# cruiseresearchgroup/ViLCo

Hardware: AMD Instinct MI355X
Metric: clips/sec (fwd+bwd) MQ transformer T=2304 C=2304 (higher is better)
Workload: dtype fp16 MFMA on 2-part splits of power-of-two scaled fp32 operands (22 significant bits, 3 MFMAs per product), fp32 accumulate: fp32-equivalent; weight-gradient products with contraction length >= 2048 use the leading fp16 parts only (11-bit operands, 1 MFMA; <= 3.5e-4 of the 3-MFMA gradients at this c; 1 GPU; MQ ViLCo backbone config P: T=2304 Cin=2304 D=1024 H=16 arch(2,2,5) XLNet layer text L=77x768 22 classes, train mode with the reference's dropout 0.1 / droppath 0.1 / XLNet dropout 0.1 (mq_vilco.yaml, xlnet_config_1024.json); clips_per_gpu=2, global_batch=2, parallelism=dp1

## Files before the change

include/vilco_hip.h:

```cpp
#ifndef VILCO_HIP_H
#define VILCO_HIP_H

#include <stddef.h>
#include <stdint.h>

#ifdef __cplusplus
extern "C" {
#endif

enum vilco_status {
  VILCO_OK = 0,
  VILCO_ERR_BADARG = -1,
  VILCO_ERR_UNSUPPORTED = -2,
  VILCO_ERR_LAUNCH = -3,
  VILCO_ERR_WORKSPACE = -4
};

const char* vilco_status_str(int status);
const char* vilco_version(void);
int vilco_sync_timeouts_read(void);

enum { VILCO_ACT_NONE = 0, VILCO_ACT_RELU = 1, VILCO_ACT_GELU = 2 };
enum { VILCO_TAP_NONE = 0, VILCO_TAP_A = 1, VILCO_TAP_B = 2 };

typedef struct vilco_gemm_desc {
  const float* A;
  const float* B;
  float* C;
  int32_t M, N, K;
  int32_t a_kcontig;
  int32_t b_kcontig;
  int64_t lda, ldb, ldc;
  int32_t batch_outer, batch_inner;
  int64_t sAo, sAi, sBo, sBi, sCo, sCi;
  int32_t tap_operand, tapC, tapT;
  int32_t precision;
  float alpha, beta;
  const float* bias;
  float* preact;
  int32_t act;
  const int32_t* row_len;
  int32_t rowT;
  const float* colscale;
  const float* residual;
  int32_t res_masked;
  void* workspace;
  size_t workspace_bytes;
  const void* a_planes;
  const void* b_planes;
  int32_t band, bandT;
  float drop_p;
  uint32_t drop_seed;
  float* amax_out;
  const float* a_amax; int32_t a_namax;
  const float* b_amax; int32_t b_namax;
  int32_t a_planes_seq, b_planes_seq;
  const float* row_mask;
} vilco_gemm_desc;

size_t vilco_gemm_workspace(const vilco_gemm_desc* d);
int vilco_gemm(const vilco_gemm_desc* d, void* stream);
int vilco_gemm_group(const vilco_gemm_desc* descs, int32_t n, void* stream);

int vilco_gemm_force(int32_t bm, int32_t ks);
int vilco_gemm_set_fixup(int32_t on);
int vilco_gemm_set_gl(int32_t on);
int vilco_gemm_set_tail128(int32_t on);
int vilco_gemm_set_skinny(int32_t on);
int64_t vilco_gemm_config_gen(void);
int32_t vilco_gemm_amax_parts(const vilco_gemm_desc* desc);
int vilco_gemm_profile_begin(void);
int vilco_gemm_profile_end(double* kernel_ms, int64_t* launches);
int64_t vilco_gemm_profile_records(int64_t* desc, double* ms, int64_t cap);

size_t vilco_pack_bytes(int64_t rows, int64_t cols, int32_t precision);
int vilco_pack(const float* src, int64_t rows, int64_t cols, int64_t ld, int32_t precision, void* planes,
               size_t planes_bytes, void* stream);
typedef struct vilco_pack_item {
  const float* src;
  int64_t rows, cols, ld;
  void* planes;
  size_t planes_bytes;
  int32_t nbatch;
  int64_t batch_stride;
  int32_t relshift;
  const float* amax;
  int32_t namax;
  int32_t seq_len;
} vilco_pack_item;
size_t vilco_pack_item_bytes(const vilco_pack_item* item, int32_t precision);
int vilco_pack_many(const vilco_pack_item* items, int32_t n, int32_t precision, void* stream);

int vilco_layernorm_fwd(const float* x, const float* gamma, const float* beta, float* y,
                        float* mean, float* rstd, int64_t rows, int32_t C, float eps,
                        int32_t relu, void* stream);
int vilco_layernorm_fwd_amax(const float* x, const float* gamma, const float* beta, float* y,
                             float* mean, float* rstd, int64_t rows, int32_t C, float eps,
                             int32_t relu, float* amax_parts, int32_t* n_parts, void* stream);
size_t vilco_layernorm_planes_bytes(int64_t rows, int32_t C, int32_t seq_len);
int vilco_layernorm_fwd_planes(const float* x, const float* gamma, const float* beta, float* y,
                               float* mean, float* rstd, int64_t rows, int32_t C, float eps,
                               int32_t relu, float* amax_parts, int32_t* n_parts, void* planes, size_t planes_bytes,
                               int32_t seq_len, const float* row_mask, int64_t mask_rows, void* stream);
size_t vilco_layernorm_bwd_workspace(int64_t rows, int32_t C);
int vilco_layernorm_bwd(const float* dy, const float* x, const float* y, const float* gamma,
                        const float* mean, const float* rstd, float* dx, float* dgamma,
                        float* dbeta, int64_t rows, int32_t C, int32_t relu, void* workspace,
                        size_t workspace_bytes, void* stream);
int vilco_layernorm_bwd_res(const float* dy, const float* x, const float* y, const float* gamma,
                            const float* mean, const float* rstd, const float* dres, float* dx, float* dgamma,
                            float* dbeta, int64_t rows, int32_t C, int32_t relu, void* workspace,
                            size_t workspace_bytes, void* stream);
int vilco_layernorm_bwd_res_amax(const float* dy, const float* x, const float* y, const float* gamma,
                                 const float* mean, const float* rstd, const float* dres, float* dx, float* dgamma,
                                 float* dbeta, int64_t rows, int32_t C, int32_t relu, void* workspace,
                                 size_t workspace_bytes, float* dx_amax_parts, int32_t* n_parts, void* stream);

int vilco_dwconv3_fwd(const float* x, const float* w, const int32_t* in_len, float* y, int32_t B,
                      int32_t Tin, int32_t C, int32_t stride, void* stream);
size_t vilco_dwconv3_bwd_workspace(int32_t B, int32_t Tin, int32_t C, int32_t stride);
int vilco_dwconv3_bwd(const float* dy, const float* x, const float* w, const int32_t* in_len,
// ... 201 lines not shown
```

vilco_amd/_lib.py:

```python
import ctypes as C
import os

_HERE = os.path.dirname(os.path.abspath(__file__))
LIB_PATH = os.environ.get("VILCO_HIP_LIB") or os.path.join(_HERE, "libvilco_hip.so")

ACT_NONE, ACT_RELU, ACT_GELU = 0, 1, 2
TAP_NONE, TAP_A, TAP_B = 0, 1, 2

c_fp = C.c_void_p
i32, i64, f32, sz = C.c_int32, C.c_int64, C.c_float, C.c_size_t


class GemmDesc(C.Structure):
    _fields_ = [
        ("A", c_fp), ("B", c_fp), ("C", c_fp),
        ("M", i32), ("N", i32), ("K", i32),
        ("a_kcontig", i32), ("b_kcontig", i32),
        ("lda", i64), ("ldb", i64), ("ldc", i64),
        ("batch_outer", i32), ("batch_inner", i32),
        ("sAo", i64), ("sAi", i64), ("sBo", i64), ("sBi", i64), ("sCo", i64), ("sCi", i64),
        ("tap_operand", i32), ("tapC", i32), ("tapT", i32),
        ("precision", i32),
        ("alpha", f32), ("beta", f32),
        ("bias", c_fp), ("preact", c_fp), ("act", i32),
        ("row_len", c_fp), ("rowT", i32),
        ("colscale", c_fp), ("residual", c_fp), ("res_masked", i32),
        ("workspace", c_fp), ("workspace_bytes", sz),
        ("a_planes", c_fp), ("b_planes", c_fp),
        ("band", i32), ("bandT", i32),
        ("drop_p", f32), ("drop_seed", C.c_uint32),
        ("amax_out", c_fp),
        ("a_amax", c_fp), ("a_namax", i32), ("b_amax", c_fp), ("b_namax", i32),
        ("a_planes_seq", i32), ("b_planes_seq", i32),
        ("row_mask", c_fp),
    ]


class LossDesc(C.Structure):
    _fields_ = [("logits", c_fp), ("offsets", c_fp), ("level_scale", c_fp), ("points", c_fp), ("row_level", c_fp),
                ("row_pos", c_fp), ("level_len", c_fp), ("gt", c_fp), ("gauss", c_fp), ("loss_norm", c_fp),
                ("B", i32), ("R", i32), ("C", i32), ("L", i32), ("Nmax", i32),
                ("center_radius", f32), ("label_smoothing", f32), ("momentum", f32), ("loss_weight", f32),
                ("al_weight", f32), ("use_al", i32)]


class AttnAmaxIn(C.Structure):
    _fields_ = [("q", c_fp), ("nq", i32), ("k", c_fp), ("nk", i32), ("v", c_fp), ("nv", i32), ("dout", c_fp), ("ndo", i32)]


class PackItem(C.Structure):
    _fields_ = [("src", c_fp), ("rows", i64), ("cols", i64), ("ld", i64), ("planes", c_fp), ("planes_bytes", sz),
                ("nbatch", i32), ("batch_stride", i64), ("relshift", i32), ("amax", c_fp), ("namax", i32), ("seq_len", i32)]


SIGNATURES = {
    "vilco_status_str": (C.c_char_p, [C.c_int]),
    "vilco_version": (C.c_char_p, []),
    "vilco_sync_timeouts_read": (C.c_int, []),
    "vilco_defer_set": (C.c_int, [i32]),
    "vilco_defer_pending": (i64, []),
    "vilco_defer_flush": (C.c_int, [c_fp]),
    "vilco_gemm_workspace": (sz, [C.POINTER(GemmDesc)]),
    "vilco_gemm": (C.c_int, [C.POINTER(GemmDesc), c_fp]),
    "vilco_gemm_group": (C.c_int, [C.POINTER(GemmDesc), i32, c_fp]),
    "vilco_gemm_amax_parts": (i32, [C.POINTER(GemmDesc)]),
    "vilco_gemm_force": (C.c_int, [i32, i32]),
    "vilco_gemm_set_fixup": (C.c_int, [i32]),
    "vilco_gemm_set_gl": (C.c_int, [i32]),
    "vilco_gemm_set_tail128": (C.c_int, [i32]),
    "vilco_gemm_set_skinny": (C.c_int, [i32]),
    "vilco_gemm_config_gen": (i64, []),
    "vilco_gemm_profile_begin": (C.c_int, []),
    "vilco_gemm_profile_end": (C.c_int, [C.POINTER(C.c_double), C.POINTER(C.c_int64)]),
    "vilco_gemm_profile_records": (C.c_int64, [C.POINTER(C.c_int64), C.POINTER(C.c_double), C.c_int64]),
    "vilco_pack_bytes": (sz, [i64, i64, i32]),
    "vilco_pack_item_bytes": (sz, [C.POINTER(PackItem), i32]),
    "vilco_pack": (C.c_int, [c_fp, i64, i64, i64, i32, c_fp, sz, c_fp]),
    "vilco_pack_many": (C.c_int, [C.POINTER(PackItem), i32, i32, c_fp]),
    "vilco_layernorm_fwd": (C.c_int, [c_fp, c_fp, c_fp, c_fp, c_fp, c_fp, i64, i32, f32, i32, c_fp]),
    "vilco_layernorm_fwd_amax": (C.c_int, [c_fp, c_fp, c_fp, c_fp, c_fp, c_fp, i64, i32, f32, i32, c_fp, C.POINTER(i32), c_fp]),
    "vilco_layernorm_planes_bytes": (sz, [i64, i32, i32]),
    "vilco_layernorm_fwd_planes": (C.c_int, [c_fp, c_fp, c_fp, c_fp, c_fp, c_fp, i64, i32, f32, i32, c_fp, C.POINTER(i32), c_fp, sz,
                                             i32, c_fp, i64, c_fp]),
    "vilco_layernorm_bwd_workspace": (sz, [i64, i32]),
    "vilco_layernorm_bwd": (C.c_int, [c_fp, c_fp, c_fp, c_fp, c_fp, c_fp, c_fp, c_fp, c_fp, i64, i32,
                                      i32, c_fp, sz, c_fp]),
    "vilco_layernorm_bwd_res": (C.c_int, [c_fp, c_fp, c_fp, c_fp, c_fp, c_fp, c_fp, c_fp, c_fp, c_fp, i64, i32,
                                          i32, c_fp, sz, c_fp]),
    "vilco_layernorm_bwd_res_amax": (C.c_int, [c_fp, c_fp, c_fp, c_fp, c_fp, c_fp, c_fp, c_fp, c_fp, c_fp, i64, i32,
                                               i32, c_fp, sz, c_fp, C.POINTER(i32), c_fp]),
    "vilco_dwconv3_fwd": (C.c_int, [c_fp, c_fp, c_fp, c_fp, i32, i32, i32, i32, c_fp]),
    "vilco_dwconv3_bwd_workspace": (sz, [i32, i32, i32, i32]),
    "vilco_dwconv3_bwd": (C.c_int, [c_fp, c_fp, c_fp, c_fp, c_fp, c_fp, i32, i32, i32, i32, c_fp, sz, c_fp]),
    "vilco_maxpool3s2_fwd": (C.c_int, [c_fp, c_fp, c_fp, i32, i32, i32, c_fp]),
    "vilco_maxpool3s2_bwd": (C.c_int, [c_fp, c_fp, c_fp, c_fp, i32, i32, i32, c_fp]),
    "vilco_softmax_fwd": (C.c_int, [c_fp, c_fp, i32, i32, i32, i32, i32, c_fp]),
    "vilco_softmax_bwd": (C.c_int, [c_fp, c_fp, i32, i32, i32, i32, c_fp]),
    "vilco_relshift_add": (C.c_int, [c_fp, c_fp, f32, i32, i32, i32, c_fp]),
    "vilco_relshift_bwd": (C.c_int, [c_fp, c_fp, f32, i32, i32, i32, c_fp]),
    "vilco_attn_supported": (C.c_int, [i32]),
    "vilco_attn_fwd_workspace": (sz, [i32, i32, i32, i32, i32, i32]),
    "vilco_attn_amax_parts": (i32, [i32, i32, i32, i32, i32, i32, i32, f32, i32]),
    "vilco_attn_fwd": (C.c_int, [c_fp, c_fp, c_fp, c_fp, c_fp, c_fp, c_fp, i32, i32, i32, i32, i32, f32, i32, i32, i32, f32,
                                 C.c_uint32, C.POINTER(AttnAmaxIn), c_fp, c_fp, sz, c_fp]),
    "vilco_attn_fwd_planes": (C.c_int, [c_fp, c_fp, c_fp, c_fp, c_fp, c_fp, c_fp, i32, i32, i32, i32, i32, f32, i32, i32, i32, f32,
                                        C.c_uint32, C.POINTER(AttnAmaxIn), c_fp, c_fp, sz, c_fp, sz, c_fp]),
    "vilco_attn_planes_supported": (i32, [i32, i32, i32, i32, i32, i32, f32]),
    "vilco_attn_bwd_workspace": (sz, [i32, i32, i32, i32, i32, i32]),
    "vilco_attn_bwd": (C.c_int, [c_fp, c_fp, c_fp, c_fp, c_fp, c_fp, c_fp, c_fp, c_fp, c_fp, c_fp, c_fp, i32, i32,
                                 i32, i32, i32, f32, i32, i32, i32, f32, C.c_uint32, C.POINTER(AttnAmaxIn), c_fp, c_fp, c_fp, c_fp, c_fp, sz,
                                 c_fp]),
    "vilco_attn_dsplanes_bytes": (sz, [i32, i32, i32]),
    "vilco_xl_scores_workspace": (sz, [i32, i32, i32, i32]),
    "vilco_xl_scores": (C.c_int, [c_fp, c_fp, c_fp, i32, i32, i32, i32, i32, i32, c_fp, sz, c_fp]),
    "vilco_attn_bwd_dsplanes": (C.c_int, [c_fp, c_fp, c_fp, c_fp, c_fp, c_fp, c_fp, c_fp, c_fp, c_fp, c_fp, c_fp, i32, i32,
                                          i32, i32, i32, f32, i32, i32, i32, f32, C.c_uint32, C.POINTER(AttnAmaxIn), c_fp, c_fp, c_fp, c_fp,
                                          c_fp, sz, c_fp, sz, c_fp]),
    "vilco_decode_workspace": (sz, [i32, i32]),
    "vilco_decode": (C.c_int, [c_fp, c_fp, c_fp, c_fp, c_fp, i32, i32, i32, f32, f32, c_fp, c_fp, c_fp, c_fp, c_fp, sz, c_fp]),
    "vilco_scale_add_fwd": (C.c_int, [c_fp, c_fp, c_fp, c_fp, c_fp, c_fp, i32, i32, i32, i32, c_fp]),
    "vilco_colsum_workspace": (sz, [i64, i32]),
    "vilco_scale_add_bwd": (C.c_int, [c_fp, c_fp, c_fp, c_fp, c_fp, i32, c_fp, c_fp, c_fp, i32, i32, i32,
                                      c_fp, sz, c_fp]),
# ... 85 lines not shown
```

vilco_amd/csrc/gemm.hip:

```cpp
#include <cstdlib>
#include <mutex>
#include <utility>
#include <vector>
#include <type_traits>
#include "common.h"
#define VILCO_TU "gemm"
#include "pack.h"

namespace {

constexpr int BN = 128, BK = 32;
constexpr int EPI_LD = 68;

__device__ __forceinline__ int swz(int row) { return (4 - ((row >> 2) & 3)) & 3; }
__device__ __forceinline__ int lds_off(int row, int chunk) { return row * 32 + ((chunk ^ swz(row)) << 3); }

struct Epi {
  float alpha, beta;
  const float* bias;
  float* preact;
  int act;
  const int* row_len;
  int rowT;
  const float* colscale;
// ... 576 lines not shown
        mem_phase2(t + 1, std::true_type{});
        __builtin_amdgcn_sched_barrier(0);
        __syncthreads();
      }
      if (t < nk) {
        if (t > 0) mfma_phase();
        __builtin_amdgcn_sched_barrier(0);
        mem_phase2(t, std::false_type{});
        __builtin_amdgcn_sched_barrier(0);
        __syncthreads();
      }
      if (nk > 0) mfma_phase();
    }
  } else
  if (!late) {
    for (int t = 0; t < nk; ++t) {
      STAMP(0);
      mem_phase(t);
#if VILCO_GEMM_VARIANT == 0 || VILCO_GEMM_VARIANT == 2
      asm volatile("s_waitcnt lgkmcnt(0)" ::: "memory");
#endif
      __builtin_amdgcn_sched_barrier(0);
      STAMP(3);
      mfma_phase();
      __builtin_amdgcn_sched_barrier(0);
      STAMP(5);
      __syncthreads();
      STAMP(6);
    }
  } else {
    for (int t = 0; t < nk; ++t) {
      STAMP(0);
      if (t > 0) mfma_phase();
      __builtin_amdgcn_sched_barrier(0);
      STAMP(3);
      mem_phase(t);
#if VILCO_GEMM_VARIANT == 0 || VILCO_GEMM_VARIANT == 2
      asm volatile("s_waitcnt lgkmcnt(0)" ::: "memory");
#endif
      __builtin_amdgcn_sched_barrier(0);
      STAMP(5);
      __syncthreads();
      STAMP(6);
    }
    if (nk > 0) mfma_phase();
  }
  STAMPX(2);

  gemm_epilogue<MI, F16, true>(g, acc, smem_raw, tid, lane, wave, wm, wn, m0, n0, bid, ks, zo, zi, (int)blockIdx.z);
  STAMPX(3);
}


template <int BM, bool AKM, bool BKM, bool SINGLE>
__device__ __forceinline__ void gemm_gl_body(const GArgs& g, const int z) {
  constexpr int MI = BM / 64;
  constexpr int A_BYTES = BM * 128, B_BYTES = BN * 128;
  constexpr int SLOT = A_BYTES + B_BYTES, STAGE = 2 * SLOT;
  constexpr int KSLOT = 64;
  constexpr int KINT = SINGLE ? 128 : 64;
  constexpr int NA0 = AKM ? 8 * ((BM / 2 + 63) / 64) : BM / 16;
  constexpr int NA1 = BM / 8 - NA0;
  constexpr int NP0 = (NA0 + 16) / 4, NP0A = NA0 / 4;
  constexpr int NP1 = NA1 / 4;
  static_assert(NA0 % 4 == 0 && NA1 % 4 == 0 && NP1 >= 1, "piece split");
  extern __shared__ __attribute__((aligned(16))) unsigned char smem_raw[];

  const int tid = threadIdx.x, lane = tid & 63;
  const int wave = __builtin_amdgcn_readfirstlane(tid >> 6);
  const int wm = wave >> 1, wn = wave & 1;
  const bool late = wave >= 4;
  const int w4 = wave & 3;
#ifdef VILCO_LAB
  const bool stamp_on = blockIdx.x == 0 && blockIdx.y == 0 && blockIdx.z == 0 && (wave & 3) == 0;
#endif
  STAMPX(0);

  int bid = blockIdx.x;
  {
    const int nwg = g.ntiles, q = nwg >> 3, r = nwg & 7, x = bid & 7;
    bid = (x < r ? x * (q + 1) : r * (q + 1) + (x - r) * q) + (bid >> 3);
  }
  const int tm = bid / g.tiles_n + g.tm0, tn = bid % g.tiles_n;
  const int m0 = tm * BM, n0 = tn * BN;
  const int zo = z / g.batch_inner, zi = z % g.batch_inner;
  const int ks = blockIdx.y;

  const __bf16* pa = g.a.p + ((long)(g.a.has_o ? zo : 0) * g.a.nbi + (g.a.has_i ? zi : 0)) * g.a.batch_stride;
  const __bf16* pb = g.b.p + ((long)(g.b.has_o ? zo : 0) * g.b.nbi + (g.b.has_i ? zi : 0)) * g.b.batch_stride;
  __amdgpu_buffer_rsrc_t rsA[2], rsB[2];
  {
    const unsigned na = g.a.bytes > 0xffffffffL ? 0xffffffffu : (unsigned)g.a.bytes;
    const unsigned nb = g.b.bytes > 0xffffffffL ? 0xffffffffu : (unsigned)g.b.bytes;
#pragma unroll
    for (int q = 0; q < 2; ++q) {
      rsA[q] = __builtin_amdgcn_make_buffer_rsrc(const_cast<__bf16*>(pa + (SINGLE ? 0 : q * g.a.plane_stride)), 0, na, 0x00020000);
      rsB[q] = __builtin_amdgcn_make_buffer_rsrc(const_cast<__bf16*>(pb + (SINGLE ? 0 : q * g.b.plane_stride)), 0, nb, 0x00020000);
    }
  }
  STAMPX(5);
  unsigned voff[NP0];
  int ldso[NP0];
  {
    const int sr = lane >> 3, cp = lane & 7;
#pragma unroll
    for (int j = 0; j < NP0; ++j) {
      const bool isB = !late && j >= NP0A;
// ... 99 lines not shown

  bf16x8 fa[2][2][MI], fb[2][2][4];
  auto reads = [&](int st) {
    const unsigned char* sbase = smem_raw + st * STAGE;
#pragma unroll
    for (int u = 0; u < 2; ++u)
#pragma unroll
      for (int h = 0; h < 2; ++h) {
#pragma unroll
        for (int i = 0; i < MI; ++i) {
          if (AKM) fa[u][h][i] = tr_frag(reinterpret_cast<const __bf16*>(sbase + u * SLOT + faddr[i] + h * fa_h1), 4 * 64);
          else fa[u][h][i] = *reinterpret_cast<const bf16x8*>(sbase + u * SLOT + (faddr[i] ^ (h * fa_h1)));
        }
#pragma unroll
        for (int j = 0; j < 4; ++j) {
          if (BKM) fb[u][h][j] = tr_frag(reinterpret_cast<const __bf16*>(sbase + u * SLOT + fbddr[j] + h * fb_h1), 4 * 64);
          else fb[u][h][j] = *reinterpret_cast<const bf16x8*>(sbase + u * SLOT + (fbddr[j] ^ (h * fb_h1)));
        }
      }
  };
  auto mfmas = [&](int nsub) {
    __builtin_amdgcn_s_setprio(1);
#pragma unroll
    for (int u = 0; u < (SINGLE ? 2 : 1); ++u)
#pragma unroll
      for (int h = 0; h < 2; ++h) {
        if ((SINGLE ? 2 * u + h : h) < nsub) {
#pragma unroll
          for (int i = 0; i < MI; ++i)
#pragma unroll
            for (int j = 0; j < 4; ++j) acc[i][j] = mma<true>(fa[u][h][i], fb[u][h][j], acc[i][j]);
          if constexpr (!SINGLE) {
#pragma unroll
            for (int i = 0; i < MI; ++i)
#pragma unroll
              for (int j = 0; j < 4; ++j) {
                acc[i][j] = mma<true>(fa[0][h][i], fb[1][h][j], acc[i][j]);
                acc[i][j] = mma<true>(fa[1][h][i], fb[0][h][j], acc[i][j]);
              }
          }
        }
      }
    __builtin_amdgcn_s_setprio(0);
  };
#define GL_BARRIER()                                  \
  do {                                                \
    __builtin_amdgcn_sched_barrier(0);                \
    __builtin_amdgcn_s_barrier();                     \
    __builtin_amdgcn_sched_barrier(0);                \
  } while (0)
#define GL_WAIT_DMA() asm volatile("s_waitcnt vmcnt(0)" ::: "memory")
#define GL_WAIT_LDS() asm volatile("s_waitcnt lgkmcnt(0)" ::: "memory")

  if (nc > 0) {
    issue(c0, 0);
    STAMPX(4);
    GL_WAIT_DMA();
    GL_BARRIER();
    STAMPX(1);
    if (!late) {
      for (int t = 0; t < nc; ++t) {
        STAMP(0);
        reads(t & 1);
        __builtin_amdgcn_sched_barrier(0);
#ifdef VILCO_LAB_FINE
        STAMP(1);
#endif
        if (t + 1 < nc) issue(c0 + t + 1, (t + 1) & 1);
        __builtin_amdgcn_sched_barrier(0);
        STAMP(2);
        GL_WAIT_LDS();
        GL_BARRIER();
        STAMP(4);
        mfmas(t + 1 < nc ? SUB : last_sub);
        __builtin_amdgcn_sched_barrier(0);
        STAMP(5);
        GL_WAIT_DMA();
        STAMP(6);
        GL_BARRIER();
        STAMP(7);
      }
    } else {
      for (int t = 0; t < nc; ++t) {
        STAMP(0);
        if (t > 0) mfmas(SUB);
        __builtin_amdgcn_sched_barrier(0);
        STAMP(1);
        GL_WAIT_DMA();
        STAMP(2);
        GL_BARRIER();
        STAMP(3);
        reads(t & 1);
        __builtin_amdgcn_sched_barrier(0);
#ifdef VILCO_LAB_FINE
        STAMP(4);
#endif
        if (t + 1 < nc) issue(c0 + t + 1, (t + 1) & 1);
        __builtin_amdgcn_sched_barrier(0);
        STAMP(5);
        GL_WAIT_LDS();
        GL_BARRIER();
        STAMP(7);
      }
      mfmas(last_sub);
    }
  }
#undef GL_BARRIER
#undef GL_WAIT_DMA
#undef GL_WAIT_LDS
  STAMPX(2);
  gemm_epilogue<MI, true, false>(g, acc, smem_raw, tid, lane, wave, wm, wn, m0, n0, bid, ks, zo, zi, z);
  STAMPX(3);
}

template <int BM, bool AKM, bool BKM, bool SINGLE>
__global__ __launch_bounds__(512) void gemm_gl_kernel(GArgs g) {
  gemm_gl_body<BM, AKM, BKM, SINGLE>(g, (int)blockIdx.z);
}

struct GArgsN { GArgs g[4]; };
template <int BM, bool AKM, bool BKM>
__global__ __launch_bounds__(512) void gemm_gl_group_kernel(GArgsN gg) {
  gemm_gl_body<BM, AKM, BKM, false>(gg.g[blockIdx.z], 0);
}


constexpr int SK_LD = 68;
template <int BMS>
__global__ __launch_bounds__(512) void gemm_skinny_kernel(GArgs g) {
  constexpr int MB = BMS / 16;
  extern __shared__ __attribute__((aligned(16))) unsigned char smem_raw[];
  float* part = reinterpret_cast<float*>(smem_raw);
  const int tid = threadIdx.x, lane = tid & 63;
  const int wave = __builtin_amdgcn_readfirstlane(tid >> 6);
  const int tiles_n = (g.N + 63) >> 6;
  const int tm = blockIdx.x / tiles_n, tn = blockIdx.x % tiles_n;
  const int m0 = tm * BMS, n0 = tn * 64;
  const int nk32 = g.Kp / BK;
  const int per = (nk32 + 7) >> 3;
  const int s0 = wave * per;
  int s1 = s0 + per;
  if (s1 > nk32) s1 = nk32;
  const int r16 = lane & 15, kq = (lane >> 4) * 8;
  const __bf16* ap[MB];
  const __bf16* bp[4];
#pragma unroll
  for (int i = 0; i < MB; ++i) ap[i] = g.a.p + row_off(g.a, m0 + 16 * i + r16) + kq;
#pragma unroll
  for (int j = 0; j < 4; ++j) bp[j] = g.b.p + row_off(g.b, n0 + 16 * j + r16) + kq;
  const long pa1 = g.a.plane_stride, pb1 = g.b.plane_stride;

  f32x4 acc[MB][4];
#pragma unroll
  for (int i = 0; i < MB; ++i)
#pragma unroll
    for (int j = 0; j < 4; ++j) acc[i][j] = f32x4{0.f, 0.f, 0.f, 0.f};
  constexpr int NB = 4;
  bf16x8 fa[NB][2][MB], fb[NB][2][4];
  for (int st = s0; st < s1; st += NB) {
#pragma unroll
    for (int u = 0; u < NB; ++u) {
      if (st + u < s1) {
        const int k = (st + u) * BK;
#pragma unroll
        for (int i = 0; i < MB; ++i) {
          fa[u][0][i] = *reinterpret_cast<const bf16x8*>(ap[i] + k);
          fa[u][1][i] = *reinterpret_cast<const bf16x8*>(ap[i] + pa1 + k);
        }
#pragma unroll
        for (int j = 0; j < 4; ++j) {
          fb[u][0][j] = *reinterpret_cast<const bf16x8*>(bp[j] + k);
          fb[u][1][j] = *reinterpret_cast<const bf16x8*>(bp[j] + pb1 + k);
        }
      }
    }
#pragma unroll
// ... 139 lines not shown
  int a_nbo, a_nbi, b_nbo, b_nbi;
  long a_bytes, b_bytes, part_bytes;
  long split_stride;
  bool tapkm;
  bool k2;
  bool fixup;
  bool gl;
  bool skinny;
};

constexpr int FIX_TILES = 4096, FIX_STREAMS = 32;
__device__ unsigned vilco_tile_counters[FIX_STREAMS * FIX_TILES];
inline bool& skinny_enabled() {
  static bool on = [] { const char* e = getenv("VILCO_GEMM_SKINNY"); return !(e && e[0] == '0'); }();
  return on;
}
inline int skinny_max_rows() {
  static const int v = [] { const char* e = getenv("VILCO_GEMM_SKINNY_M"); const int x = e ? atoi(e) : 640; return x > 0 ? x : 640; }();
  return v;
}
inline int skinny_bm16_rows() {
  static const int v = [] { const char* e = getenv("VILCO_GEMM_SKINNY_BM16"); const int x = e ? atoi(e) : 640; return x >= 0 ? x : 640; }();
  return v;
}
inline int skinny_max_k() {
  static const int v = [] { const char* e = getenv("VILCO_GEMM_SKINNY_K"); const int x = e ? atoi(e) : 768; return x > 0 ? x : 768; }();
  return v;
}
inline bool& fixup_enabled() {
  static bool on = [] { const char* e = getenv("VILCO_GEMM_FIXUP"); return e && e[0] == '1'; }();
  return on;
}
unsigned* tile_counters(hipStream_t s) {
  static std::mutex mu;
  static hipStream_t streams[FIX_STREAMS];
  static int n = 0;
  static unsigned* base = nullptr;
  std::lock_guard<std::mutex> lk(mu);
  if (!base) {
    void* q = nullptr;
    if (hipGetSymbolAddress(&q, HIP_SYMBOL(vilco_tile_counters)) != hipSuccess || !q) return nullptr;
    base = reinterpret_cast<unsigned*>(q);
  }
  for (int i = 0; i < n; ++i)
    if (streams[i] == s) return base + (long)i * FIX_TILES;
  if (n >= FIX_STREAMS) return nullptr;
  streams[n] = s;
  return base + (long)(n++) * FIX_TILES;
}

inline bool& gl_enabled() {
  static bool v = [] { const char* e = getenv("VILCO_GEMM_GL"); return !(e && e[0] == '0'); }();
  return v;
}

inline bool& tail128_enabled() {
  static bool v = [] { const char* e = getenv("VILCO_GEMM_TAIL128"); return e && e[0] == '1'; }();
  return v;
}

inline bool tapkm_enabled() {
  static const bool v = [] { const char* e = getenv("VILCO_CONV_DW_KM"); return !(e && e[0] == '0'); }();
  return v;
}

void make_plan(const vilco_gemm_desc* d, Plan& p) {
  p.NP = d->precision == 1 ? 1 : ((d->precision == 0 || d->precision == 3 || d->precision == 4) ? 2 : 3);
  p.Kp = (int)align_up(d->K > 0 ? d->K : 1, 32);
  p.a_tr = !d->a_kcontig;
  p.b_tr = !d->b_kcontig;
  p.a_tap = p.b_tap = 0;
  p.tapkm = false;
  p.a_out_rows = d->M;
  p.b_out_rows = d->N;
  long a_batch = (long)d->M * p.Kp, b_batch = (long)d->N * p.Kp;
  const bool km_ok = use_km() && d->tap_operand == VILCO_TAP_NONE;
  p.a_km = km_ok && p.a_tr;
  p.b_km = km_ok && p.b_tr;
  if (p.a_km) { p.a_tr = false; p.a_out_rows = p.Kp; a_batch = (long)p.Kp * align_up(d->M, 32); }
  if (p.b_km) { p.b_tr = false; p.b_out_rows = p.Kp; b_batch = (long)p.Kp * align_up(d->N, 32); }
  if (d->tap_operand == VILCO_TAP_A) {
    if ((d->tapC % 8) == 0) {
      p.a_tap = 1;
      const long nseq = d->M / d->tapT;
      const long slack = (p.Kp + d->tapC - 1) / d->tapC;
      p.a_out_rows = (int)(nseq * (d->tapT + 2) + slack);
      a_batch = (long)p.a_out_rows * d->tapC;
    } else {
      p.a_tap = 2;
    }
  } else if (d->tap_operand == VILCO_TAP_B) {
    if (use_km() && tapkm_enabled() && (d->tapC % 8) == 0 && (d->M % 8) == 0 && d->tapT > 0 && (d->K % d->tapT) == 0 &&
        d->batch_outer == 1 && d->batch_inner == 1) {
      const long nseq = d->K / d->tapT;
      p.tapkm = true;
      p.Kp = (int)align_up(nseq * (d->tapT + 2) - 1, 32);
      p.a_tap = p.b_tap = 1;
      p.a_tr = p.b_tr = false;
      p.a_km = p.b_km = true;
      p.a_out_rows = p.Kp + 1 + 32;
      p.b_out_rows = p.Kp + 3 + 32;
      a_batch = (long)p.a_out_rows * d->M;
      b_batch = (long)p.b_out_rows * d->tapC;
    } else {
      p.b_tap = 3;
    }
// ... 73 lines not shown
      if (k > 16) k = 16;
      if (k < 1) k = 1;
      const double m = model(bms[q], k, cs[q]);
      if (m < best_t) { best_t = m; best_bm = bms[q]; best_ks = k; }
    }
    if (best_bm != 128 && best_t <= 0.92 * base) { p.BM = best_bm; ks = best_ks; }
  }
  const int force_bm = tune().bm, force_ks = tune().ks;
  if (force_bm == 128 || (force_bm == 256 && !p.gl) || (force_bm == 192 && d->precision >= 3)) p.BM = force_bm;
  if (force_ks >= 1 && force_ks <= nk) ks = force_ks;
  p.skinny = false;
  if (skinny_enabled() && force_bm == 0 && force_ks < 1 && d->precision == 3 && gl_enabled() && !p.a_tr && !p.b_tr && !p.a_km && !p.b_km &&
      d->tap_operand == VILCO_TAP_NONE && d->band == 0 && nbatch == 1 && d->M <= skinny_max_rows() && d->K >= 64 && d->K <= skinny_max_k() &&
      d->N <= 1024) {
    p.skinny = true;
    p.gl = false;
    p.BM = d->M <= skinny_bm16_rows() ? 16 : 32;
    ks = 1;
  }
  p.kchunk = (nk + ks - 1) / ks;
  p.ksplit = (nk + p.kchunk - 1) / p.kchunk;
  long out_span = 0;
  if (p.ksplit > 1) {
    out_span = (long)(d->batch_outer - 1) * d->sCo + (long)(d->batch_inner - 1) * d->sCi + (long)(d->M - 1) * d->ldc + d->N;
    out_span = align_up(out_span, 64);
  }
  p.split_stride = out_span;
  p.part_bytes = p.ksplit > 1 ? align_up(out_span * p.ksplit * 4, 256) : 0;
  p.fixup = false;
  if (p.ksplit > 1 && fixup_enabled() && !p.gl) {
    const long ntiles = tn * ((d->M + p.BM - 1) / p.BM) * nbatch;
    if (ntiles <= FIX_TILES) {
      p.fixup = true;
      p.part_bytes = align_up(ntiles * p.ksplit * (long)p.BM * BN * 4, 256);
    }
  }
}

template <int BM, int NP, bool F16, bool AKM, bool BKM, bool K2 = false>
void launch_pp_km(const GArgs& g, dim3 grid, hipStream_t s) {
  constexpr size_t a_el = AKM ? 32 * ((BM == 192 ? 256 : BM) + 16) : BM * 32, b_el = BKM ? 32 * (BN + 16) : BN * 32;
  constexpr size_t pipe = (size_t)2 * NP * (a_el + b_el) * sizeof(__bf16), epi = (size_t)8 * 16 * (BM / 64) * EPI_LD * 4;
  constexpr size_t lds = pipe > epi ? pipe : epi;
  static const bool once = [] {
    hipFuncSetAttribute(reinterpret_cast<const void*>(&gemm_pp_kernel<BM, NP, F16, AKM, BKM, K2>),
                        hipFuncAttributeMaxDynamicSharedMemorySize, (int)lds);
    (void)hipGetLastError();
    return true;
  }();
  (void)once;
  hipLaunchKernelGGL((gemm_pp_kernel<BM, NP, F16, AKM, BKM, K2>), grid, dim3(512), lds, s, g);
}

template <int BM, bool AKM, bool BKM, bool SINGLE>
void launch_gl_km(const GArgs& g, dim3 grid, hipStream_t s) {
  constexpr size_t lds = (size_t)4 * (BM + BN) * 128;
  static const bool once = [] {
    hipFuncSetAttribute(reinterpret_cast<const void*>(&gemm_gl_kernel<BM, AKM, BKM, SINGLE>),
                        hipFuncAttributeMaxDynamicSharedMemorySize, (int)lds);
    (void)hipGetLastError();
    return true;
  }();
  (void)once;
  hipLaunchKernelGGL((gemm_gl_kernel<BM, AKM, BKM, SINGLE>), grid, dim3(512), lds, s, g);
}
template <int BM, bool SINGLE>
void launch_gl(const GArgs& g, dim3 grid, hipStream_t s, bool akm, bool bkm) {
  if (akm && bkm) launch_gl_km<BM, true, true, SINGLE>(g, grid, s);
  else if (bkm) launch_gl_km<BM, false, true, SINGLE>(g, grid, s);
  else launch_gl_km<BM, false, false, SINGLE>(g, grid, s);
}

template <int BM, int NP, bool F16 = false, bool K2 = false>
void launch_pp(const GArgs& g, dim3 grid, hipStream_t s, bool akm = false, bool bkm = false) {
  if (akm && bkm) launch_pp_km<BM, NP, F16, true, true, K2>(g, grid, s);
  else if (bkm) launch_pp_km<BM, NP, F16, false, true, K2>(g, grid, s);
  else launch_pp_km<BM, NP, F16, false, false, K2>(g, grid, s);
}

}

#ifdef VILCO_LAB
extern "C" int vilco_lab_read(unsigned long long* out) {
  return (int)hipMemcpyFromSymbol(out, HIP_SYMBOL(vilco_lab_stamps), sizeof(unsigned long long) * 2 * 64 * 8);
}
#endif

namespace {
template <int BMS>
static void launch_skinny(const GArgs& g, hipStream_t s) {
  constexpr size_t lds = (size_t)8 * BMS * SK_LD * 4;
  static const bool once = [] {
    hipFuncSetAttribute(reinterpret_cast<const void*>(&gemm_skinny_kernel<BMS>), hipFuncAttributeMaxDynamicSharedMemorySize, (int)lds);
    (void)hipGetLastError();
    return true;
  }();
  (void)once;
  const int tiles = ((g.N + 63) / 64) * ((g.M + BMS - 1) / BMS);
  hipLaunchKernelGGL((gemm_skinny_kernel<BMS>), dim3(tiles), dim3(512), lds, s, g);
}

struct ProfRec { int64_t v[10]; };
struct ProfState {
  bool on = false;
  std::vector<std::pair<hipEvent_t, hipEvent_t>> ev;
  std::vector<ProfRec> rec;
  std::vector<double> ms;
};
ProfState& prof() { static ProfState p; return p; }
}

static long amax_out_parts(const vilco_gemm_desc* d, const Plan& p) {
  const long nz = (long)d->batch_outer * d->batch_inner;
  if (p.ksplit > 1 && !p.fixup) {
    long blocks = ((long)d->M * d->N * nz + 255) / 256;
    return blocks > 2048 ? 2048 : blocks;
  }
  if (p.skinny) return (long)((d->N + 63) / 64) * ((d->M + p.BM - 1) / p.BM);
  const long n = (long)((d->N + BN - 1) / BN) * ((d->M + p.BM - 1) / p.BM) * nz;
  return n <= 8192 ? n : 0;
}

extern "C" int32_t vilco_gemm_amax_parts(const vilco_gemm_desc* d) {
// ... 316 lines not shown
  hipEvent_t ev0 = nullptr, ev1 = nullptr;
  if (prof().on) { hipEventCreate(&ev0); hipEventCreate(&ev1); hipEventRecord(ev0, s); }
  {
    const bool ak = p.a_km, bk = p.b_km;
    if (p.skinny) {
      if (p.BM == 16) launch_skinny<16>(g, s); else launch_skinny<32>(g, s);
    } else if (p.gl) {
      const bool single = d->precision == 4;
      if (p.BM == 192) { if (single) launch_gl<192, true>(g, grid, s, ak, bk); else launch_gl<192, false>(g, grid, s, ak, bk); }
      else { if (single) launch_gl<128, true>(g, grid, s, ak, bk); else launch_gl<128, false>(g, grid, s, ak, bk); }
    } else if (d->precision == 4 && p.k2) {
      if (p.BM == 256) launch_pp<256, 2, true, true>(g, grid, s, ak, bk);
      else if (p.BM == 192) launch_pp<192, 2, true, true>(g, grid, s, ak, bk);
      else launch_pp<128, 2, true, true>(g, grid, s, ak, bk);
    } else if (d->precision == 4) {
      if (p.BM == 256) launch_pp<256, 1, true>(g, grid, s, ak, bk);
      else if (p.BM == 192) launch_pp<192, 1, true>(g, grid, s, ak, bk);
      else launch_pp<128, 1, true>(g, grid, s, ak, bk);
    } else if (f16) {
      if (p.BM == 256) launch_pp<256, 2, true>(g, grid, s, ak, bk);
      else if (p.BM == 192) launch_pp<192, 2, true>(g, grid, s, ak, bk);
      else launch_pp<128, 2, true>(g, grid, s, ak, bk);
    }
    else if (p.BM == 256) {
      if (p.NP == 1) launch_pp<256, 1>(g, grid, s, ak, bk);
      else if (p.NP == 2) launch_pp<256, 2>(g, grid, s, ak, bk);
      else launch_pp<256, 3>(g, grid, s, ak, bk);
    } else {
      if (p.NP == 1) launch_pp<128, 1>(g, grid, s, ak, bk);
      else if (p.NP == 2) launch_pp<128, 2>(g, grid, s, ak, bk);
      else launch_pp<128, 3>(g, grid, s, ak, bk);
    }
  }
  if (ev0) {
    hipEventRecord(ev1, s);
    prof().ev.emplace_back(ev0, ev1);
    prof().rec.push_back(ProfRec{{d->M, d->N, d->K, nz, p.BM, p.ksplit, d->precision, p.a_km, p.b_km, p.a_tap | (p.b_tap << 4)}});
  }
  if (p.ksplit > 1 && !p.fixup && vilco_defer_active() && nz == 1 && d->alpha == 1.f && d->beta == 0.f && !d->bias &&
      !d->preact && d->act == VILCO_ACT_NONE && !d->row_len && !d->row_mask && !d->colscale && !d->residual && d->drop_p == 0.f &&
      !d->amax_out) {
    vilco_defer_push_sk(g.c, g.cfinal, g.split_stride, g.ldc, d->M, d->N, p.ksplit);
  } else if (p.ksplit > 1 && !p.fixup) {
    long blocks = ((long)d->M * d->N * nz + 255) / 256;
    if (blocks > 2048) blocks = 2048;
    if (g.vec_out) hipLaunchKernelGGL(splitk_reduce_kernel<true>, dim3((int)blocks), dim3(256), 0, s, g, nz);
    else hipLaunchKernelGGL(splitk_reduce_kernel<false>, dim3((int)blocks), dim3(256), 0, s, g, nz);
  }
  return vilco_launch_status();
}

extern "C" int vilco_gemm(const vilco_gemm_desc* d, void* stream) { return gemm_impl(d, stream, nullptr, nullptr); }

template <int BM>
static void launch_gl_group(const GArgsN& gg, int n, int ntiles, hipStream_t s, bool akm, bool bkm) {
  constexpr size_t lds = (size_t)4 * (BM + BN) * 128;
  const dim3 grid(ntiles, 1, n);
#define VILCO_GROUP_LAUNCH(A_, B_)                                                                                      \
  do {                                                                                                                  \
    static const bool once = [] {                                                                                       \
      hipFuncSetAttribute(reinterpret_cast<const void*>(&gemm_gl_group_kernel<BM, A_, B_>),                             \
                          hipFuncAttributeMaxDynamicSharedMemorySize, (int)lds);                                        \
      (void)hipGetLastError();                                                                                          \
      return true;                                                                                                      \
    }();                                                                                                                \
    (void)once;                                                                                                         \
    hipLaunchKernelGGL((gemm_gl_group_kernel<BM, A_, B_>), grid, dim3(512), lds, s, gg);                                \
  } while (0)
  if (akm && bkm) VILCO_GROUP_LAUNCH(true, true);
  else if (bkm) VILCO_GROUP_LAUNCH(false, true);
  else VILCO_GROUP_LAUNCH(false, false);
#undef VILCO_GROUP_LAUNCH
}

extern "C" int vilco_gemm_group(const vilco_gemm_desc* descs, int32_t n, void* stream) {
  if (!descs || n < 1 || n > 4) return VILCO_ERR_BADARG;
  static const bool enabled = [] { const char* e = getenv("VILCO_GEMM_GROUP"); return !(e && e[0] == '0'); }();
  hipStream_t s = reinterpret_cast<hipStream_t>(stream);
  GArgsN gg;
  Plan p0;
  bool ok = enabled && n >= 2;
  for (int i = 0; ok && i < n; ++i) {
    const vilco_gemm_desc& d = descs[i];
    Plan p;
    ok = d.precision == 3 && d.batch_outer == 1 && d.batch_inner == 1 && d.tap_operand == VILCO_TAP_NONE && d.band == 0 &&
         d.M == descs[0].M && d.N == descs[0].N && d.K == descs[0].K && d.a_kcontig == descs[0].a_kcontig &&
         d.b_kcontig == descs[0].b_kcontig && d.M > 0 && d.N > 0 && gemm_impl(&d, stream, &gg.g[i], &p) == VILCO_OK &&
         p.gl && p.ksplit == 1 && (i == 0 || (p.BM == p0.BM && p.a_km == p0.a_km && p.b_km == p0.b_km));
    if (i == 0) p0 = p;
  }
  if (!ok) {
    for (int i = 0; i < n; ++i) {
      const int rc = vilco_gemm(&descs[i], stream);
      if (rc != VILCO_OK) return rc;
    }
    return VILCO_OK;
  }
  hipEvent_t ev0 = nullptr, ev1 = nullptr;
  if (prof().on) { hipEventCreate(&ev0); hipEventCreate(&ev1); hipEventRecord(ev0, s); }
  if (p0.BM == 192) launch_gl_group<192>(gg, n, gg.g[0].ntiles, s, p0.a_km, p0.b_km);
  else launch_gl_group<128>(gg, n, gg.g[0].ntiles, s, p0.a_km, p0.b_km);
  if (ev0) {
    hipEventRecord(ev1, s);
    prof().ev.emplace_back(ev0, ev1);
    prof().rec.push_back(ProfRec{{descs[0].M, descs[0].N, descs[0].K, n, p0.BM, 1, 3, p0.a_km, p0.b_km, 0x100}});
  }
  return vilco_launch_status();
}

static int64_t g_config_gen = 0;
extern "C" int64_t vilco_gemm_config_gen(void) { return g_config_gen; }

extern "C" int vilco_gemm_set_fixup(int32_t on) {
  fixup_enabled() = on != 0;
  ++g_config_gen;
  return VILCO_OK;
}

extern "C" int vilco_gemm_set_gl(int32_t on) {
  gl_enabled() = on != 0;
  ++g_config_gen;
  return VILCO_OK;
}

extern "C" int vilco_gemm_set_skinny(int32_t on) {
  skinny_enabled() = on != 0;
  ++g_config_gen;
  return VILCO_OK;
}

extern "C" int vilco_gemm_set_tail128(int32_t on) {
  tail128_enabled() = on != 0;
  ++g_config_gen;
  return VILCO_OK;
}

extern "C" int vilco_gemm_force(int32_t bm, int32_t ks) {
  if (bm < 0 || ks < 0) return VILCO_ERR_BADARG;
  tune().bm = bm; tune().ks = ks;
  ++g_config_gen;
  return VILCO_OK;
}
```

Baseline: 99.55 clips/s.

## Add deep multi-slot LDS ring pipeline to split-precision GL GEMM

Adds a RING variant of the GL GEMM body that fills up to 160KB of LDS with a ring of 3-5 k-slices fed by direct buffer-to-LDS loads. Each wave issues DMA several slices ahead and waits on a graded vmcnt, so MFMAs on the hi and lo parts overlap deeper prefetch. It is chosen by default for non-single GEMMs with at least 6 k-chunks and at most 256 workgroups, and also for grouped launches. The larger LDS footprint lowers occupancy, and the new hand-coded waitcnt logic risks correctness or stalls.

```diff
diff --git a/include/vilco_hip.h b/include/vilco_hip.h
--- a/include/vilco_hip.h
+++ b/include/vilco_hip.h
@@ -67,6 +67,7 @@
 int vilco_gemm_set_gl(int32_t on);
 int vilco_gemm_set_tail128(int32_t on);
 int vilco_gemm_set_skinny(int32_t on);
+int vilco_gemm_set_ring(int32_t on);
 int64_t vilco_gemm_config_gen(void);
 int32_t vilco_gemm_amax_parts(const vilco_gemm_desc* desc);
 int vilco_gemm_profile_begin(void);
diff --git a/vilco_amd/_lib.py b/vilco_amd/_lib.py
--- a/vilco_amd/_lib.py
+++ b/vilco_amd/_lib.py
@@ -69,6 +69,7 @@
     "vilco_gemm_set_gl": (C.c_int, [i32]),
     "vilco_gemm_set_tail128": (C.c_int, [i32]),
     "vilco_gemm_set_skinny": (C.c_int, [i32]),
+    "vilco_gemm_set_ring": (C.c_int, [i32]),
     "vilco_gemm_config_gen": (i64, []),
     "vilco_gemm_profile_begin": (C.c_int, []),
     "vilco_gemm_profile_end": (C.c_int, [C.POINTER(C.c_double), C.POINTER(C.c_int64)]),
diff --git a/vilco_amd/csrc/gemm.hip b/vilco_amd/csrc/gemm.hip
--- a/vilco_amd/csrc/gemm.hip
+++ b/vilco_amd/csrc/gemm.hip
@@ -652,7 +652,13 @@
 }
 
 
-template <int BM, bool AKM, bool BKM, bool SINGLE>
+__device__ __forceinline__ void gl_dma16(__amdgpu_buffer_rsrc_t rs, const unsigned char* lds, unsigned voff, int soff) {
+  const unsigned m = __builtin_amdgcn_readfirstlane((unsigned)(uintptr_t)(__attribute__((address_space(3))) const void*)lds);
+  asm volatile("s_mov_b32 m0, %0\n\ts_nop 0\n\tbuffer_load_dwordx4 %1, %2, %3 offen lds" ::"s"(m), "v"(voff), "s"(rs), "s"(soff) : "memory");
+}
+constexpr int GL_LDS_BYTES = 160 * 1024;
+#define GL_RING_SLOTS(BM) (GL_LDS_BYTES / (((BM) + BN) * 128))
+template <int BM, bool AKM, bool BKM, bool SINGLE, bool RING>
 __device__ __forceinline__ void gemm_gl_body(const GArgs& g, const int z) {
   constexpr int MI = BM / 64;
   constexpr int A_BYTES = BM * 128, B_BYTES = BN * 128;
@@ -858,6 +864,159 @@
 #define GL_WAIT_DMA() asm volatile("s_waitcnt vmcnt(0)" ::: "memory")
 #define GL_WAIT_LDS() asm volatile("s_waitcnt lgkmcnt(0)" ::: "memory")
 
+  if constexpr (RING && !SINGLE) {
+    constexpr int NSLOT = GL_RING_SLOTS(BM), L = NSLOT - 1;
+    constexpr int PER0 = NP0, PER1 = NP1;
+    const int total = 2 * nc;
+    auto slot_base = [&](int s) { return smem_raw + (s % NSLOT) * SLOT; };
+    auto issue1 = [&](auto part_, int s) {
+      constexpr int u = decltype(part_)::value;
+      unsigned char* sbase = slot_base(s);
+      const int kc64 = c0 + (s >> 1);
+      const int sa = kc64 * kstepA, sb = kc64 * kstepB;
+      if (!late) {
+#pragma unroll
+        for (int j = 0; j < NP0; ++j) gl_dma16(j >= NP0A ? rsB[u] : rsA[u], sbase + ldso[j], voff[j], j >= NP0A ? sb : sa);
+      } else {
+#pragma unroll
+        for (int j = 0; j < NP1; ++j) gl_dma16(rsA[u], sbase + ldso[j], voff[j], sa);
+      }
+    };
+    auto reads1 = [&](auto part_, int s) {
+      constexpr int u = decltype(part_)::value;
+      const unsigned char* sbase = slot_base(s);
+#pragma unroll
+      for (int h = 0; h < 2; ++h) {
+#pragma unroll
+        for (int i = 0; i < MI; ++i) {
+          if (AKM) fa[u][h][i] = tr_frag(reinterpret_cast<const __bf16*>(sbase + faddr[i] + h * fa_h1), 4 * 64);
+          else fa[u][h][i] = *reinterpret_cast<const bf16x8*>(sbase + (faddr[i] ^ (h * fa_h1)));
+        }
+#pragma unroll
+        for (int j = 0; j < 4; ++j) {
+          if (BKM) fb[u][h][j] = tr_frag(reinterpret_cast<const __bf16*>(sbase + fbddr[j] + h * fb_h1), 4 * 64);
+          else fb[u][h][j] = *reinterpret_cast<const bf16x8*>(sbase + (fbddr[j] ^ (h * fb_h1)));
+        }
+      }
+    };
+    auto mfma_hi = [&]() {
+      __builtin_amdgcn_s_setprio(1);
+#pragma unroll
+      for (int i = 0; i < MI; ++i)
+#pragma unroll
+        for (int j = 0; j < 4; ++j) acc[i][j] = mma<true>(fa[0][0][i], fb[0][0][j], acc[i][j]);
+      __builtin_amdgcn_s_setprio(0);
+    };
+    auto mfma_lo = [&](int nsub) {
+      __builtin_amdgcn_s_setprio(1);
+#pragma unroll
+      for (int h = 0; h < 2; ++h)
+        if (h < nsub) {
+          if (h > 0) {
+#pragma unroll
+            for (int i = 0; i < MI; ++i)
+#pragma unroll
+              for (int j = 0; j < 4; ++j) acc[i][j] = mma<true>(fa[0][h][i], fb[0][h][j], acc[i][j]);
+          }
+#pragma unroll
+          for (int i = 0; i < MI; ++i)
+#pragma unroll
+            for (int j = 0; j < 4; ++j) {
+              acc[i][j] = mma<true>(fa[0][h][i], fb[1][h][j], acc[i][j]);
+              acc[i][j] = mma<true>(fa[1][h][i], fb[0][h][j], acc[i][j]);
+            }
+        }
+      __builtin_amdgcn_s_setprio(0);
+    };
+    auto wait_next = [&](int s) {
+      const int k = total - 2 - s;
+      if (!late) {
+        if (k >= L - 1) asm volatile("s_waitcnt vmcnt(%0)" ::"n"((L - 1) * PER0) : "memory");
+        else if (L > 3 && k == 2) asm volatile("s_waitcnt vmcnt(%0)" ::"n"(2 * PER0) : "memory");
+        else if (k == 1) asm volatile("s_waitcnt vmcnt(%0)" ::"n"(PER0) : "memory");
+        else asm volatile("s_waitcnt vmcnt(0)" ::: "memory");
+      } else {
+        if (k >= L - 1) asm volatile("s_waitcnt vmcnt(%0)" ::"n"((L - 1) * PER1) : "memory");
+        else if (L > 3 && k == 2) asm volatile("s_waitcnt vmcnt(%0)" ::"n"(2 * PER1) : "memory");
+        else if (k == 1) asm volatile("s_waitcnt vmcnt(%0)" ::"n"(PER1) : "memory");
+        else asm volatile("s_waitcnt vmcnt(0)" ::: "memory");
+      }
+    };
+    static_assert(NSLOT >= 3 && NSLOT <= 5, "wait_next covers leads of 2..4");
+    using P0 = std::integral_constant<int, 0>;
+    using P1 = std::integral_constant<int, 1>;
+    using PL = std::integral_constant<int, L & 1>;
+    using PL1 = std::integral_constant<int, (L + 1) & 1>;
+    if (nc > 0) {
+#pragma unroll
+      for (int q = 0; q < L; ++q)
+        if (q < total) { if (q & 1) issue1(P1{}, q); else issue1(P0{}, q); }
+      STAMPX(4);
+      wait_next(-1);
+      GL_BARRIER();
+      STAMPX(1);
+      if (!late) {
+        for (int t = 0; t < nc; ++t) {
+          const int s = 2 * t, nsub = t + 1 < nc ? SUB : last_sub;
+          STAMP(0);
+          reads1(P0{}, s);
+          __builtin_amdgcn_sched_barrier(0);
+          if (s + L < total) issue1(PL{}, s + L);
+          __builtin_amdgcn_sched_barrier(0);
+          GL_WAIT_LDS();
+          GL_BARRIER();
+          mfma_hi();
+          __builtin_amdgcn_sched_barrier(0);
+          STAMP(2);
+          wait_next(s);
+          GL_BARRIER();
+          STAMP(4);
+          reads1(P1{}, s + 1);
+          __builtin_amdgcn_sched_barrier(0);
+          if (s + 1 + L < total) issue1(PL1{}, s + 1 + L);
+          __builtin_amdgcn_sched_barrier(0);
+          GL_WAIT_LDS();
+          GL_BARRIER();
+          mfma_lo(nsub);
+          __builtin_amdgcn_sched_barrier(0);
+          STAMP(6);
+          wait_next(s + 1);
+          GL_BARRIER();
+          STAMP(7);
+        }
+      } else {
+        for (int t = 0; t < nc; ++t) {
+          const int s = 2 * t, nsub = t + 1 < nc ? SUB : last_sub;
+          STAMP(0);
+          if (t > 0) mfma_lo(SUB);
+          __builtin_amdgcn_sched_barrier(0);
+          wait_next(s - 1);
+          GL_BARRIER();
+          STAMP(2);
+          reads1(P0{}, s);
+          __builtin_amdgcn_sched_barrier(0);
+          if (s + L < total) issue1(PL{}, s + L);
+          __builtin_amdgcn_sched_barrier(0);
+          GL_WAIT_LDS();
+          GL_BARRIER();
+          STAMP(4);
+          mfma_hi();
+          __builtin_amdgcn_sched_barrier(0);
+          wait_next(s);
+          GL_BARRIER();
+          STAMP(6);
+          reads1(P1{}, s + 1);
+          __builtin_amdgcn_sched_barrier(0);
+          if (s + 1 + L < total) issue1(PL1{}, s + 1 + L);
+          __builtin_amdgcn_sched_barrier(0);
+          GL_WAIT_LDS();
+          GL_BARRIER();
+          STAMP(7);
+        }
+        mfma_lo(last_sub);
+      }
+    }
+  } else
   if (nc > 0) {
     issue(c0, 0);
     STAMPX(4);
@@ -919,15 +1078,15 @@
   STAMPX(3);
 }
 
-template <int BM, bool AKM, bool BKM, bool SINGLE>
+template <int BM, bool AKM, bool BKM, bool SINGLE, bool RING>
 __global__ __launch_bounds__(512) void gemm_gl_kernel(GArgs g) {
-  gemm_gl_body<BM, AKM, BKM, SINGLE>(g, (int)blockIdx.z);
+  gemm_gl_body<BM, AKM, BKM, SINGLE, RING>(g, (int)blockIdx.z);
 }
 
 struct GArgsN { GArgs g[4]; };
-template <int BM, bool AKM, bool BKM>
+template <int BM, bool AKM, bool BKM, bool RING>
 __global__ __launch_bounds__(512) void gemm_gl_group_kernel(GArgsN gg) {
-  gemm_gl_body<BM, AKM, BKM, false>(gg.g[blockIdx.z], 0);
+  gemm_gl_body<BM, AKM, BKM, false, RING>(gg.g[blockIdx.z], 0);
 }
 
 
@@ -1173,6 +1332,15 @@
 inline bool& gl_enabled() {
   static bool v = [] { const char* e = getenv("VILCO_GEMM_GL"); return !(e && e[0] == '0'); }();
   return v;
+}
+
+constexpr int GL_RING_MIN_CHUNKS = 6;
+inline int& ring_mode() {
+  static int v = [] { const char* e = getenv("VILCO_GEMM_RING"); return e ? atoi(e) : 1; }();
+  return v;
+}
+inline bool use_ring(const GArgs& g, long wgs) {
+  return ring_mode() == 2 || (ring_mode() == 1 && g.kchunk >= GL_RING_MIN_CHUNKS && wgs <= 256);
 }
 
 inline bool& tail128_enabled() {
@@ -1352,23 +1520,31 @@
   hipLaunchKernelGGL((gemm_pp_kernel<BM, NP, F16, AKM, BKM, K2>), grid, dim3(512), lds, s, g);
 }
 
-template <int BM, bool AKM, bool BKM, bool SINGLE>
+template <int BM, bool RING>
+constexpr size_t gl_lds_bytes() { return RING ? (size_t)GL_RING_SLOTS(BM) * (BM + BN) * 128 : (size_t)4 * (BM + BN) * 128; }
+template <int BM, bool AKM, bool BKM, bool SINGLE, bool RING>
 void launch_gl_km(const GArgs& g, dim3 grid, hipStream_t s) {
-  constexpr size_t lds = (size_t)4 * (BM + BN) * 128;
+  constexpr size_t lds = gl_lds_bytes<BM, RING>();
+  static_assert(lds <= GL_LDS_BYTES, "gemm_gl LDS");
   static const bool once = [] {
-    hipFuncSetAttribute(reinterpret_cast<const void*>(&gemm_gl_kernel<BM, AKM, BKM, SINGLE>),
+    hipFuncSetAttribute(reinterpret_cast<const void*>(&gemm_gl_kernel<BM, AKM, BKM, SINGLE, RING>),
                         hipFuncAttributeMaxDynamicSharedMemorySize, (int)lds);
     (void)hipGetLastError();
     return true;
   }();
   (void)once;
-  hipLaunchKernelGGL((gemm_gl_kernel<BM, AKM, BKM, SINGLE>), grid, dim3(512), lds, s, g);
+  hipLaunchKernelGGL((gemm_gl_kernel<BM, AKM, BKM, SINGLE, RING>), grid, dim3(512), lds, s, g);
+}
+template <int BM, bool SINGLE, bool RING = false>
+void launch_gl_o(const GArgs& g, dim3 grid, hipStream_t s, bool akm, bool bkm) {
+  if (akm && bkm) launch_gl_km<BM, true, true, SINGLE, RING>(g, grid, s);
+  else if (bkm) launch_gl_km<BM, false, true, SINGLE, RING>(g, grid, s);
+  else launch_gl_km<BM, false, false, SINGLE, RING>(g, grid, s);
 }
 template <int BM, bool SINGLE>
 void launch_gl(const GArgs& g, dim3 grid, hipStream_t s, bool akm, bool bkm) {
-  if (akm && bkm) launch_gl_km<BM, true, true, SINGLE>(g, grid, s);
-  else if (bkm) launch_gl_km<BM, false, true, SINGLE>(g, grid, s);
-  else launch_gl_km<BM, false, false, SINGLE>(g, grid, s);
+  if (!SINGLE && use_ring(g, (long)grid.x * grid.y * grid.z)) launch_gl_o<BM, false, true>(g, grid, s, akm, bkm);
+  else launch_gl_o<BM, SINGLE>(g, grid, s, akm, bkm);
 }
 
 template <int BM, int NP, bool F16 = false, bool K2 = false>
@@ -1791,25 +1967,30 @@
 
 extern "C" int vilco_gemm(const vilco_gemm_desc* d, void* stream) { return gemm_impl(d, stream, nullptr, nullptr); }
 
-template <int BM>
-static void launch_gl_group(const GArgsN& gg, int n, int ntiles, hipStream_t s, bool akm, bool bkm) {
-  constexpr size_t lds = (size_t)4 * (BM + BN) * 128;
+template <int BM, bool RING>
+static void launch_gl_group_r(const GArgsN& gg, int n, int ntiles, hipStream_t s, bool akm, bool bkm) {
+  constexpr size_t lds = gl_lds_bytes<BM, RING>();
   const dim3 grid(ntiles, 1, n);
 #define VILCO_GROUP_LAUNCH(A_, B_)                                                                                      \
   do {                                                                                                                  \
     static const bool once = [] {                                                                                       \
-      hipFuncSetAttribute(reinterpret_cast<const void*>(&gemm_gl_group_kernel<BM, A_, B_>),                             \
+      hipFuncSetAttribute(reinterpret_cast<const void*>(&gemm_gl_group_kernel<BM, A_, B_, RING>),                             \
                           hipFuncAttributeMaxDynamicSharedMemorySize, (int)lds);                                        \
       (void)hipGetLastError();                                                                                          \
       return true;                                                                                                      \
     }();                                                                                                                \
     (void)once;                                                                                                         \
-    hipLaunchKernelGGL((gemm_gl_group_kernel<BM, A_, B_>), grid, dim3(512), lds, s, gg);                                \
+    hipLaunchKernelGGL((gemm_gl_group_kernel<BM, A_, B_, RING>), grid, dim3(512), lds, s, gg);                                \
   } while (0)
   if (akm && bkm) VILCO_GROUP_LAUNCH(true, true);
   else if (bkm) VILCO_GROUP_LAUNCH(false, true);
   else VILCO_GROUP_LAUNCH(false, false);
 #undef VILCO_GROUP_LAUNCH
+}
+template <int BM>
+static void launch_gl_group(const GArgsN& gg, int n, int ntiles, hipStream_t s, bool akm, bool bkm) {
+  if (use_ring(gg.g[0], (long)ntiles * n)) launch_gl_group_r<BM, true>(gg, n, ntiles, s, akm, bkm);
+  else launch_gl_group_r<BM, false>(gg, n, ntiles, s, akm, bkm);
 }
 
 extern "C" int vilco_gemm_group(const vilco_gemm_desc* descs, int32_t n, void* stream) {
@@ -1868,6 +2049,13 @@
   return VILCO_OK;
 }
 
+extern "C" int vilco_gemm_set_ring(int32_t mode) {
+  if (mode < 0 || mode > 2) return VILCO_ERR_BADARG;
+  ring_mode() = mode;
+  ++g_config_gen;
+  return VILCO_OK;
+}
+
 extern "C" int vilco_gemm_set_tail128(int32_t on) {
   tail128_enabled() = on != 0;
   ++g_config_gen;
```

Result: no change. 100.0 clips/s, median of 6 (+0.5%).
